# jrnerupudinho/Semi-Blind-Channel-Estimation-for-MIMO-RIS-communication-system-Using-EM-Algo

Hardware: NVIDIA B200
Metric: EM channel-estimation trials/sec (higher is better)
Workload: dtype f64

## Files before the change

### semi-blind-channel-estimation-for-mimo-ris-communication-system-using-em-algo_b200/csrc/abi.cu

```cuda
#include <atomic>
#include <mutex>
#include <vector>
#include <stdio.h>
#include <string.h>

#include "common.cuh"

namespace sbce {

static std::atomic<long long> g_launches{0};
void count_launch(int n) { g_launches.fetch_add(n, std::memory_order_relaxed); }

struct PhaseSpan { int phase; cudaEvent_t a, b; };
static std::atomic<bool> g_prof_on{false};
static std::vector<PhaseSpan> g_spans;
static std::vector<cudaEvent_t> g_event_pool;
static std::mutex g_prof_mu;

static cudaEvent_t prof_event() {
    {
        std::lock_guard<std::mutex> lock(g_prof_mu);
        if (!g_event_pool.empty()) { cudaEvent_t e = g_event_pool.back(); g_event_pool.pop_back(); return e; }
    }
    cudaEvent_t e;
    cudaEventCreate(&e);
    return e;
}

struct PhaseScope {
    bool on; int phase; cudaStream_t s; cudaEvent_t a;
    PhaseScope(int ph, cudaStream_t st) : on(g_prof_on.load(std::memory_order_relaxed)), phase(ph), s(st), a(nullptr) {
        if (on) { a = prof_event(); cudaEventRecord(a, s); }
    }
    ~PhaseScope() {
        if (on) {
            cudaEvent_t b = prof_event();
            cudaEventRecord(b, s);
            std::lock_guard<std::mutex> lock(g_prof_mu);
            g_spans.push_back({phase, a, b});
        }
    }
};

static int make_dims(const sbce_cfg* c, Dims* d, bool with_estep = true) {
    if (!c) return SBCE_E_NULL;
    if (c->N < 1 || c->n_tx < 1 || c->n_rx < 1 || c->T_p < 0 || c->T_d < 1 || c->itera < 0 || c->batch < 0)
        return SBCE_E_SHAPE;
    int sq = 0;
    if (c->M == 4) sq = 2; else if (c->M == 16) sq = 4; else if (c->M == 64) sq = 8; else return SBCE_E_UNSUPPORTED;
    if (c->n_tx > 8 || c->n_rx > 8) return SBCE_E_UNSUPPORTED;
    if (!gram_supports(c->N + 1, c->n_tx, c->n_rx)) return SBCE_E_UNSUPPORTED;
    if (c->n_tx <= 4 && !(c->n_rx <= 4 || c->n_rx == 6 || c->n_rx == 8)) return SBCE_E_UNSUPPORTED;
    if (c->mode < SBCE_MODE_SOFT || c->mode > SBCE_MODE_MMSE) return SBCE_E_UNSUPPORTED;
    if (with_estep) {
        const int log2M = sq == 2 ? 2 : (sq == 4 ? 4 : 6), bits = c->n_tx * log2M;
        const bool tree = c->mode == SBCE_MODE_SOFT || c->mode == SBCE_MODE_HARD;
        if (tree && !enum_instantiated(c->n_tx, log2M)) return SBCE_E_UNSUPPORTED;
        if ((c->mode == SBCE_MODE_ZF || c->mode == SBCE_MODE_MMSE) && bits > 30) return SBCE_E_UNSUPPORTED;
    }
    d->N = c->N; d->N1 = c->N + 1; d->n_tx = c->n_tx; d->n_rx = c->n_rx; d->M = c->M; d->sqM = sq;
    d->bitsM = (sq == 2 ? 2 : (sq == 4 ? 4 : 6));
    d->T_p = c->T_p; d->T_d = c->T_d; d->itera = c->itera;
    d->L = d->N1 * c->n_tx;
    d->Lp = (d->L + 7) & ~7;
    d->RP = (c->n_rx + 3) & ~3;
    d->Ltot = d->Lp + d->RP;
    d->mode = c->mode; d->flags = c->flags; d->p1 = c->partition_p1;
    d->psi_shared = (c->flags & SBCE_FLAG_PSI_SHARED) ? 1 : 0;
    d->psiP_shared = (c->flags & (SBCE_FLAG_PSI_SHARED | SBCE_FLAG_PSIP_SHARED)) ? 1 : 0;
    d->rec = qr_record_doubles(c->n_tx);
    if (c->mode == SBCE_MODE_PM || c->mode == SBCE_MODE_PM_BETA) {
        if (c->partition_p1 < 1 || c->partition_p1 > c->n_tx) return SBCE_E_SHAPE;
        if (with_estep && c->partition_p1 * d->bitsM > 24) return SBCE_E_UNSUPPORTED;
    }
    if (c->mode >= SBCE_MODE_PM && c->n_rx < c->n_tx) return SBCE_E_UNSUPPORTED;
    if (c->flags & SBCE_FLAG_SUPERIMPOSED) {
        if (c->T_p != 0) return SBCE_E_SHAPE;
        if (c->mode != SBCE_MODE_SOFT && c->mode != SBCE_MODE_HARD) return SBCE_E_UNSUPPORTED;
    }
    return 0;
}

static inline size_t al(size_t x) { return (x + 255) & ~(size_t)255; }

size_t carve_workspace(const Dims& d, int nb, void* base, Workspace* ws) {
    size_t off = 0;
    char* p = (char*)base;
    auto take = [&](size_t bytes) { char* r = p ? p + off : nullptr; off += al(bytes); return r; };
    const size_t B = (size_t)nb;
    ws->stat_m = (double*)take(B * d.T_d * d.n_tx * 16);
    ws->stat_R = (double*)take(B * d.T_d * d.n_tx * d.n_tx * 16);
    ws->pil_m = (double*)take(B * d.T_p * d.n_tx * 16 + 16);
    ws->pil_R = (double*)take(B * d.T_p * d.n_tx * d.n_tx * 16 + 16);
    ws->qr = (double*)take(B * d.T_d * d.rec * 8);
    ws->lse_sym = (double*)take(B * d.T_d * 8);
    ws->Gp = (double*)take(B * d.Ltot * d.Lp * 16);
    ws->G = (double*)take(B * d.Ltot * d.Lp * 16);
    ws->active = (int32_t*)take(B * 4);
    ws->stat = (int32_t*)take(B * 4);
    ws->kscratch = (int32_t*)take(B * d.T_d * 4);
    ws->thbuf = (double*)take(B * d.Lp * d.n_rx * 16);
    ws->psiw = (double*)take(B * d.T_p * d.N1 * 16 + 16);
    ws->ls_scale = (double*)take(B * d.N1 * 8);
    ws->ls_rep = (int32_t*)take(B * d.N1 * 4);
    ws->bytes = off;
    return off;
}

#define CK(x)                                  \
    do {                                       \
        cudaError_t _e = (x);                  \
        if (_e != cudaSuccess) return (int)_e; \
    } while (0)

cudaError_t launch_pm_stats(const Dims& d, int nb, const double* Yd, const double* PsiD, const double* theta,
                            const double* varn, const int32_t* active, double* stat_m, double* stat_R,
                            int32_t* kstar, cudaStream_t s);

static int estep_dispatch(const Dims& d, int nb, const double* Yd, const double* PsiD, const double* theta,
                          const double* varn, const int32_t* active, Workspace& ws, double* stat_m, double* stat_R,
                          int32_t* kstar, double* lse_sym, const double* Xoff, cudaStream_t s) {
    if (d.mode == SBCE_MODE_SOFT || d.mode == SBCE_MODE_HARD) {
        {
            PhaseScope ps(SBCE_PHASE_HEFF_QR, s);
            CK(launch_heff_qr(d, nb, Yd, PsiD, theta, active, Xoff, ws.qr, s));
        }
        {
            PhaseScope ps(SBCE_PHASE_ENUM, s);
            CK(launch_enum(d, nb, ws.qr, varn, active, stat_m, stat_R, kstar, lse_sym, s));
            if (Xoff) CK(launch_superimpose_stats(d, nb, Xoff, active, stat_m, stat_R, s));
        }
    } else {
        PhaseScope ps(SBCE_PHASE_ENUM, s);
        CK(launch_pm_stats(d, nb, Yd, PsiD, theta, varn, active, stat_m, stat_R, kstar, s));
    }
    return 0;
}

static inline Dims pilot_dims(const Dims& d) { Dims dp = d; dp.psi_shared = d.psiP_shared; return dp; }

static int em_chunk(const Dims& d, int nb, const sbce_io& io, Workspace& ws, cudaStream_t s) {
    const bool tree = d.mode == SBCE_MODE_SOFT || d.mode == SBCE_MODE_HARD;
    const bool decides = tree || d.mode == SBCE_MODE_ZF || d.mode == SBCE_MODE_MMSE;
    if (io.kstar && !decides) CK(cudaMemsetAsync(io.kstar, 0xFF, (size_t)nb * d.T_d * sizeof(int32_t), s));
    {
        PhaseScope ps(SBCE_PHASE_SETUP, s);
        CK(launch_init_state(d, nb, io.theta0, io.theta, ws.active, ws.stat, io.iters, io.llf, io.lse, s));
        CK(launch_pilot_stats(d, nb, io.Xp, ws.pil_m, ws.pil_R, s));
        CK(launch_normal_equations(pilot_dims(d), nb, io.PsiP, d.T_p, io.Yp, ws.pil_m, ws.pil_R, nullptr, ws.Gp, nullptr, s));
    }
    for (int l = 0; l < d.itera; ++l) {
        int rc = estep_dispatch(d, nb, io.Yd, io.PsiD, io.theta, io.varn, ws.active, ws, ws.stat_m, ws.stat_R,
                                io.kstar, ws.lse_sym, (d.flags & SBCE_FLAG_SUPERIMPOSED) ? io.Xp : nullptr, s);
        if (rc) return rc;
        {
            PhaseScope ps(SBCE_PHASE_GRAM, s);
            CK(launch_normal_equations(d, nb, io.PsiD, d.T_d, io.Yd, ws.stat_m, ws.stat_R, ws.Gp, ws.G, ws.active,
                                       s));
        }
        {
            PhaseScope ps(SBCE_PHASE_CHOL, s);
            CK(launch_chol_solve(d, nb, ws.G, io.theta, ws.active, ws.stat, ws.thbuf, s));
        }
        {
            PhaseScope ps(SBCE_PHASE_METRICS, s);
            CK(launch_after_iteration(d, nb, l, io.theta, io.h_true, io.Yp, io.Yd, io.PsiP, io.PsiD, io.Xp,
                                      io.Xd_true, io.varn, tree ? ws.lse_sym : nullptr, ws.active, io.iters, io.llf,
                                      io.lse, s));
        }
    }
    {
        PhaseScope ps(SBCE_PHASE_METRICS, s);
        CK(launch_final_metrics(d, nb, io.theta, io.h_true, ws.stat, io.nmse, io.status, s));
    }
    return 0;
}

static sbce_io offset_io(const Dims& d, const sbce_io& io, size_t b0) {
    sbce_io o = io;
    const size_t Ln = (size_t)d.L * d.n_rx * 2;
    auto adv = [](const double* p, size_t n) { return p ? p + n : p; };
    auto advw = [](double* p, size_t n) { return p ? p + n : p; };
    o.Yd = adv(io.Yd, b0 * d.T_d * d.n_rx * 2);
    o.Yp = adv(io.Yp, b0 * d.T_p * d.n_rx * 2);
    if (!d.psi_shared) o.PsiD = adv(io.PsiD, b0 * d.T_d * d.N1 * 2);
    if (!d.psiP_shared) o.PsiP = adv(io.PsiP, b0 * d.T_p * d.N1 * 2);
    o.Xp = adv(io.Xp, b0 * ((d.flags & SBCE_FLAG_SUPERIMPOSED) ? d.T_d : d.T_p) * d.n_tx * 2);
    o.theta0 = adv(io.theta0, b0 * Ln);
    o.varn = adv(io.varn, b0);
    o.h_true = adv(io.h_true, b0 * Ln);
    o.Xd_true = adv(io.Xd_true, b0 * d.T_d * d.n_tx * 2);
    o.theta = advw(io.theta, b0 * Ln);
    o.kstar = io.kstar ? io.kstar + b0 * d.T_d : nullptr;
    o.llf = advw(io.llf, b0 * d.itera);
    o.lse = advw(io.lse, b0 * d.itera);
    o.nmse = advw(io.nmse, b0);
    o.iters = io.iters ? io.iters + b0 : nullptr;
    o.status = io.status ? io.status + b0 : nullptr;
    return o;
}

static int check_io(const Dims& d, const sbce_io* io) {
    if (!io) return SBCE_E_NULL;
    if (!io->Yd || !io->PsiD || !io->varn || !io->theta) return SBCE_E_NULL;
    if (d.T_p > 0 && (!io->Yp || !io->PsiP || !io->Xp)) return SBCE_E_NULL;
    if (!(d.flags & SBCE_FLAG_ZERO_START) && !io->theta0) return SBCE_E_NULL;
    if ((d.flags & SBCE_FLAG_GENIE_STOP) && !io->h_true) return SBCE_E_NULL;
    if ((d.flags & SBCE_FLAG_SUPERIMPOSED) && !io->Xp) return SBCE_E_NULL;
    return 0;
}

}

using namespace sbce;

extern "C" {

int sbce_version(void) { return SBCE_VERSION; }

const char* sbce_error_string(int code) {
    switch (code) {
        case 0: return "ok";
        case SBCE_E_NULL: return "required pointer is null";
        case SBCE_E_SHAPE: return "invalid shape parameter";
        case SBCE_E_UNSUPPORTED: return "unsupported configuration (n_tx,n_rx<=8; n_tx<=4: n_rx in {1,2,3,4,6,8}; M in {4,16,64}; N+1+n_tx^2<=908; exhaustive modes with n_tx>4 need n_tx*log2(M)<=24; PM modes need partition_p1*log2(M)<=24)";
        case SBCE_E_WORKSPACE: return "workspace too small for one trial";
        case SBCE_E_NODEVICE: return "no CUDA device";
        default: return code > 0 ? cudaGetErrorString((cudaError_t)code) : "unknown error";
    }
}

int sbce_device_count(void) {
    int n = 0;
    if (cudaGetDeviceCount(&n) != cudaSuccess) { cudaGetLastError(); return 0; }
    return n;
}

int sbce_workspace_bytes(const sbce_cfg* cfg, int32_t trials_in_flight, size_t* bytes) {
    Dims d;
    int rc = make_dims(cfg, &d);
    if (rc) return rc;
    if (!bytes) return SBCE_E_NULL;
    if (trials_in_flight < 1) return SBCE_E_SHAPE;
    Workspace ws;
    *bytes = carve_workspace(d, trials_in_flight, nullptr, &ws);
    return 0;
}

constexpr int SBCE_MAX_CHUNK = 65535;
static int trials_fitting(const Dims& d, size_t bytes, int want) {
    Workspace ws;
    if (want > SBCE_MAX_CHUNK) want = SBCE_MAX_CHUNK;
    if (carve_workspace(d, 1, nullptr, &ws) > bytes) return 0;
    int lo = 1, hi = want;
    while (lo < hi) {
        int mid = (lo + hi + 1) / 2;
        if (carve_workspace(d, mid, nullptr, &ws) <= bytes) lo = mid; else hi = mid - 1;
    }
    return lo;
}

int sbce_em_batch(const sbce_cfg* cfg, const sbce_io* io, void* workspace, size_t workspace_bytes, void* stream) {
    Dims d;
    int rc = make_dims(cfg, &d);
    if (rc) return rc;
    rc = check_io(d, io);
    if (rc) return rc;
    if (cfg->batch == 0) return 0;
    if (!workspace) return SBCE_E_NULL;
    const int chunk = trials_fitting(d, workspace_bytes, cfg->batch);
    if (chunk < 1) return SBCE_E_WORKSPACE;
    cudaStream_t s = (cudaStream_t)stream;
    for (int b0 = 0; b0 < cfg->batch; b0 += chunk) {
        const int nb = (cfg->batch - b0 < chunk) ? cfg->batch - b0 : chunk;
        Workspace ws;
        carve_workspace(d, nb, workspace, &ws);
        sbce_io o = offset_io(d, *io, (size_t)b0);
        rc = em_chunk(d, nb, o, ws, s);
        if (rc) return rc;
    }
    return 0;
}
// ... 392 lines not shown
```

### semi-blind-channel-estimation-for-mimo-ris-communication-system-using-em-algo_b200/csrc/common.cuh

```cuda
#pragma once

#include <cuda_runtime.h>
#include <stdint.h>

#include <atomic>

#include "../../include/sbce.h"

namespace sbce {

typedef double2 cplx;

__host__ __device__ __forceinline__ cplx mk(double re, double im) { return make_double2(re, im); }
__device__ __forceinline__ cplx cadd(cplx a, cplx b) { return mk(a.x + b.x, a.y + b.y); }
__device__ __forceinline__ cplx csub(cplx a, cplx b) { return mk(a.x - b.x, a.y - b.y); }
__device__ __forceinline__ cplx cmul(cplx a, cplx b) {
    return mk(fma(a.x, b.x, -a.y * b.y), fma(a.x, b.y, a.y * b.x));
}
__device__ __forceinline__ cplx cmulc(cplx a, cplx b) {
    return mk(fma(a.x, b.x, a.y * b.y), fma(a.y, b.x, -a.x * b.y));
}
__device__ __forceinline__ cplx cconj(cplx a) { return mk(a.x, -a.y); }
__device__ __forceinline__ cplx cscale(cplx a, double s) { return mk(a.x * s, a.y * s); }
__device__ __forceinline__ double cnorm2(cplx a) { return fma(a.x, a.x, a.y * a.y); }
__device__ __forceinline__ void cfma(cplx& acc, cplx a, cplx b) {
    acc.x = fma(a.x, b.x, acc.x);
    acc.x = fma(-a.y, b.y, acc.x);
    acc.y = fma(a.x, b.y, acc.y);
    acc.y = fma(a.y, b.x, acc.y);
}
__device__ __forceinline__ void cfmac(cplx& acc, cplx a, cplx b) {
    acc.x = fma(a.x, b.x, acc.x);
    acc.x = fma(a.y, b.y, acc.x);
    acc.y = fma(a.y, b.x, acc.y);
    acc.y = fma(-a.x, b.y, acc.y);
}
__device__ __forceinline__ void cfmsc(cplx& acc, cplx a, cplx b) {
    acc.x = fma(-a.x, b.x, acc.x);
    acc.x = fma(-a.y, b.y, acc.x);
    acc.y = fma(-a.y, b.x, acc.y);
    acc.y = fma(a.x, b.y, acc.y);
}

__device__ __forceinline__ double shfl_xor_d(double v, int m) { return __shfl_xor_sync(0xffffffffu, v, m); }
__device__ __forceinline__ double shfl_d(double v, int src) { return __shfl_sync(0xffffffffu, v, src); }
__device__ __forceinline__ double warp_sum(double v) {
#pragma unroll
    for (int o = 16; o > 0; o >>= 1) v += shfl_xor_d(v, o);
    return v;
}

constexpr int RH_MAXR = 8;

struct Dims {
    int N, N1, n_tx, n_rx, M, sqM, bitsM, T_p, T_d, itera;
    int L;
    int Lp;
    int RP;
    int Ltot;
    int mode;
    unsigned flags;
    int p1;
    int psi_shared;
    int psiP_shared;
    int rec;
};

__host__ __device__ __forceinline__ constexpr int qr_rec_R(int n_tx, int i, int j) {
    return 2 * (i * n_tx - i * (i - 1) / 2 + j - i);
}
__host__ __device__ __forceinline__ constexpr int qr_rec_yt(int n_tx, int i) { return n_tx * (n_tx + 1) + 2 * i; }
__host__ __device__ __forceinline__ constexpr int qr_rec_c0(int n_tx) { return qr_rec_yt(n_tx, n_tx); }
__host__ __device__ __forceinline__ constexpr int qr_record_doubles(int n_tx) { return n_tx * (n_tx + 1) + 2 * n_tx + 2; }
static_assert(qr_rec_yt(8, 0) == qr_rec_R(8, 7, 7) + 2 && qr_rec_c0(8) + 2 == qr_record_doubles(8),
              "QR record: R, ytilde and c0 are packed back to back");

constexpr bool enum_instantiated(int n_tx, int log2M) { return n_tx <= 4 || n_tx * log2M <= 24; }

struct Workspace {
    double* stat_m;
    double* stat_R;
    double* pil_m;
    double* pil_R;
    double* qr;
    double* lse_sym;
    double* Gp;
    double* G;
    int32_t* active;
    int32_t* stat;
    int32_t* kscratch;
    double* psiw;
    double* ls_scale;
    int32_t* ls_rep;
    double* thbuf;
    size_t bytes;
};

size_t carve_workspace(const Dims& d, int nb, void* base, Workspace* ws);

cudaError_t launch_pilot_stats(const Dims& d, int nb, const double* Xp, double* pil_m, double* pil_R, cudaStream_t s);
cudaError_t launch_heff_qr(const Dims& d, int nb, const double* Yd, const double* PsiD, const double* theta,
                           const int32_t* active, const double* Xoff, double* qr, cudaStream_t s);
cudaError_t launch_superimpose_stats(const Dims& d, int nb, const double* Xoff, const int32_t* active, double* stat_m,
                                     double* stat_R, cudaStream_t s);
cudaError_t launch_enum(const Dims& d, int nb, const double* qr, const double* varn, const int32_t* active,
                        double* stat_m, double* stat_R, int32_t* kstar, double* lse_sym, cudaStream_t s);
cudaError_t launch_normal_equations(const Dims& d, int nb, const double* Psi, int T, const double* Y,
                                    const double* sm, const double* sR, const double* Ginit, double* Gout,
                                    const int32_t* active, cudaStream_t s);
bool gram_supports(int N1, int n_tx, int n_rx);
cudaError_t launch_chol_solve(const Dims& d, int nb, double* G, double* theta, const int32_t* active, int32_t* stat,
                              double* th_scratch, cudaStream_t s);
cudaError_t launch_init_state(const Dims& d, int nb, const double* theta0, double* theta, int32_t* active,
                              int32_t* stat, int32_t* iters, double* llf, double* lse, cudaStream_t s);
cudaError_t launch_after_iteration(const Dims& d, int nb, int l, const double* theta, const double* h_true,
                                   const double* Yp, const double* Yd, const double* PsiP, const double* PsiD,
                                   const double* Xp, const double* Xd_true, const double* varn, const double* lse_sym,
                                   int32_t* active, int32_t* iters, double* llf, double* lse, cudaStream_t s);
cudaError_t launch_final_metrics(const Dims& d, int nb, const double* theta, const double* h_true, const int32_t* stat,
                                 double* nmse, int32_t* status, cudaStream_t s);
cudaError_t launch_accumulate_nmse(const double* nmse, const int32_t* status, int batch, double* acc, cudaStream_t s);
cudaError_t run_fp64_peak(double* tflops, double* seconds);
cudaError_t launch_generate(const Dims& d, int nb, const sbce_gen* g, const sbce_io& io, double* h_out, double* Xp_out,
                            double* Xd_out, double* PsiP_out, double* PsiD_out, double* Yp_out, double* Yd_out,
                            cudaStream_t s);
cudaError_t launch_ls_start(const Dims& d, int nb, const sbce_io& io, double* theta0, int32_t* status, Workspace& ws,
                            cudaStream_t s);
cudaError_t launch_accumulate_ser(const Dims& d, int nb, const int32_t* kstar, const double* Xd, double* acc,
                                  cudaStream_t s);

void count_launch(int n = 1);


struct SmemOptIn {
    std::atomic<size_t> have[64];
};
inline cudaError_t opt_in_smem(SmemOptIn& st, const void* kernel, size_t smem) {
    if (smem <= 48 * 1024) return cudaSuccess;
    int dev = 0;
    cudaError_t e = cudaGetDevice(&dev);
    if (e != cudaSuccess) return e;
    if (dev >= 0 && dev < 64 && st.have[dev].load(std::memory_order_relaxed) >= smem) return cudaSuccess;
    e = cudaFuncSetAttribute(kernel, cudaFuncAttributeMaxDynamicSharedMemorySize, (int)smem);
    if (e == cudaSuccess && dev >= 0 && dev < 64) st.have[dev].store(smem, std::memory_order_relaxed);
    return e;
}

}
```

### semi-blind-channel-estimation-for-mimo-ris-communication-system-using-em-algo_b200/csrc/estep.cu

```cuda
#include <math.h>

#include "common.cuh"
#include "tensor.cuh"

namespace sbce {

static __device__ __forceinline__ constexpr int cmax(int a, int b) { return a > b ? a : b; }

__global__ void k_pilot_stats(int n_tx, int total, const cplx* __restrict__ Xp, cplx* __restrict__ pm,
                              cplx* __restrict__ pR) {
    int s = blockIdx.x * blockDim.x + threadIdx.x;
    if (s >= total) return;
    const cplx* x = Xp + (size_t)s * n_tx;
    for (int i = 0; i < n_tx; ++i) {
        cplx xi = x[i];
        pm[(size_t)s * n_tx + i] = cconj(xi);
        for (int j = 0; j < n_tx; ++j) pR[((size_t)s * n_tx + i) * n_tx + j] = cmulc(x[j], xi);
    }
}

cudaError_t launch_pilot_stats(const Dims& d, int nb, const double* Xp, double* pil_m, double* pil_R, cudaStream_t s) {
    int total = nb * d.T_p;
    if (total == 0) return cudaSuccess;
    k_pilot_stats<<<(total + 127) / 128, 128, 0, s>>>(d.n_tx, total, (const cplx*)Xp, (cplx*)pil_m, (cplx*)pil_R);
// ... 526 lines not shown
        }
        __syncwarp(hm);
    }
    __syncwarp(hm);
    if (lane == 0) ws[E::O_AREF] = aref;
    __syncwarp(hm);
}

template <int NTX, int SQM, bool HARD>
struct Scan {
    typedef EnumT<NTX, SQM> E;
    static constexpr int M = E::M;
    double* ws;
    const cplx* tab;
    const double* g;
    double r0;
    double thr;
    double best, lim;
    int bestk;
    int cnt;
    bool prune;

    __device__ __forceinline__ void leaf(cplx t0, double nb, int code, bool live) {
        const double fI = E::fold(t0.x, r0), fQ = E::fold(t0.y, r0);
        const double nodemin = fma(fI, fI, fma(fQ, fQ, nb));
        const bool hit = live && nodemin <= lim;
        if (hit && nodemin <= best) {
            double dI, dQ;
            const int iI = E::slice(t0.x, g, dI), iQ = E::slice(t0.y, g, dQ);
            const double val = nb + dI + dQ;
            const int k = code + ((iQ * SQM + iI) << (E::BITS * (NTX - 1)));
            if (val < best || (val == best && k < bestk)) {
                best = val;
                bestk = k;
                lim = HARD ? val : val + thr;
            }
        }
        if (!HARD) {
            const unsigned q = __ballot_sync(E::gmask(), hit) >> E::gshift();
            if (q != 0u) {
                if (hit) {
                    const int slot = cnt + __popc(q & ((1u << E::glane()) - 1u));
                    if (slot < E::QCAP) ((int*)(ws + E::O_Q))[slot] = code;
                }
                cnt += __popc(q);
            }
        }
    }

    __device__ __forceinline__ void merge_best() {
        const unsigned hm = E::gmask();
#pragma unroll
        for (int o = E::G / 2; o > 0; o >>= 1) {
            const double ob = shfl_xor_h(hm, best, o);
            const int ok = __shfl_xor_sync(hm, bestk, o);
            if (ob < best || (ob == best && ok < bestk)) { best = ob; bestk = ok; }
        }
        lim = HARD ? best : best + thr;
    }

    template <int PER_LANE>
    __device__ __forceinline__ void maybe_flush() {
        if (!HARD && cnt > E::QCAP - E::G * PER_LANE) {
            const unsigned hm = E::gmask();
            double wb = best;
#pragma unroll
            for (int o = E::G / 2; o > 0; o >>= 1) wb = fmin(wb, shfl_xor_h(hm, wb, o));
            enum_flush<NTX, SQM>(ws, wb, cnt);
            cnt = 0;
        }
    }


    template <int S_>
    __device__ __forceinline__ void inner(const cplx (&acc)[NTX], double base, int code, cplx r01, bool dead) {
        dead = dead || (prune && base > lim);
        if constexpr (S_ == 0) {
            leaf(acc[0], base, code, !dead);
        } else if constexpr (S_ == 1 && M % E::G == 0) {
            const unsigned hm = E::gmask();
            unsigned todo = __ballot_sync(hm, !dead) >> E::gshift();
            while (todo != 0u) {
                const int src = __ffs(todo) - 1;
                todo &= todo - 1u;
                cplx pacc[NTX];
#pragma unroll
                for (int i = 0; i < NTX; ++i)
                    pacc[i] = i <= 1 ? mk(__shfl_sync(hm, acc[i].x, src, E::G), __shfl_sync(hm, acc[i].y, src, E::G))
                                     : acc[i];
                const double pbase = __shfl_sync(hm, base, src, E::G);
                const int pcode = __shfl_sync(hm, code, src, E::G);
#pragma unroll 1
                for (int m = E::glane(); m < M; m += E::G) {
                    cplx nacc[NTX];
                    const double nb = E::step(pacc, nacc, 1, m, pbase, g, tab);
                    const double b0 = best;
                    inner<0>(nacc, nb, pcode + (m << (E::BITS * (NTX - 2))), r01, false);
                    if (__any_sync(hm, best != b0)) merge_best();
                    maybe_flush<1>();
                }
            }
        } else if constexpr (S_ == 1) {
            if (__all_sync(E::gmask(), dead)) return;
            constexpr bool NODE_FLUSH = E::G * M < E::QCAP;
            const double* g1 = g + SQM;
            double dI1[SQM];
#pragma unroll
            for (int a = 0; a < SQM; ++a) {
                const double eI = acc[1].x - g1[a];
                dI1[a] = eI * eI;
            }
#pragma unroll 1
            for (int iQ = 0; iQ < SQM; ++iQ) {
                const double eQ = acc[1].y - g1[iQ];
                const double bq = base + __dmul_rn(eQ, eQ);
                const bool deadq = dead || (prune && bq > lim);
                if (__all_sync(E::gmask(), deadq)) continue;
                const double pQ = E::pam(iQ);
                const cplx tq = mk(fma(pQ, r01.y, acc[0].x), fma(-pQ, r01.x, acc[0].y));
                const int cq = code + ((iQ * SQM) << (E::BITS * (NTX - 2)));
#pragma unroll
                for (int iI = 0; iI < SQM; ++iI) {
                    const double pI = E::pam(iI);
                    const cplx t0 = mk(fma(-pI, r01.x, tq.x), fma(-pI, r01.y, tq.y));
                    leaf(t0, bq + dI1[iI], cq + (iI << (E::BITS * (NTX - 2))), !deadq);
                }
                if (!NODE_FLUSH) maybe_flush<SQM>();
            }
            if (NODE_FLUSH) maybe_flush<M>();
        } else {
            if (__all_sync(E::gmask(), dead)) return;
#pragma unroll 1
            for (int m = 0; m < M; ++m) {
                cplx nacc[NTX];
                const double nb = E::step(acc, nacc, S_, m, base, g, tab);
                inner<S_ - 1>(nacc, nb, code + (m << (E::BITS * (NTX - 1 - S_))), r01, dead);
            }
        }
    }

    template <int S_, int LEFT>
    __device__ __forceinline__ void prefix(const cplx (&acc)[NTX], double base, int code, int p, cplx r01, bool dead) {
        if constexpr (LEFT == 0) {
            inner<S_>(acc, base, code, r01, dead);
        } else {
            const int m = (p >> (E::BITS * (LEFT - 1))) & (M - 1);
            cplx nacc[NTX];
            const double nb = E::step(acc, nacc, S_, m, base, g, tab);
            prefix<S_ - 1, LEFT - 1>(nacc, nb, code + (m << (E::BITS * (NTX - 1 - S_))), p, r01, dead);
        }
    }
};

template <int NTX, int SQM, bool HARD, int WARPS>
__global__ void __launch_bounds__(WARPS * 32, (NTX > 4 ? 2 : 4)) k_enum(Dims d, const double* __restrict__ qr,
                                                     const double* __restrict__ varn,
                                                     const int32_t* __restrict__ active, cplx* __restrict__ stat_m,
                                                     cplx* __restrict__ stat_R, int32_t* __restrict__ kstar,
                                                     double* __restrict__ lse_sym) {
    typedef EnumT<NTX, SQM> E;
    constexpr int M = E::M;
    extern __shared__ __align__(16) double enum_smem[];
    const int b = blockIdx.y;
    constexpr int SPW = 32 / E::G;
    const int warp = threadIdx.x >> 5, sub = (threadIdx.x & 31) / E::G, gl = E::glane();
    const int t = (blockIdx.x * WARPS + warp) * SPW + sub;
    if (t >= d.T_d) return;
    const double* grec = qr + ((size_t)b * d.T_d + t) * d.rec;
    const int32_t act = (active != nullptr) ? active[b] : 1;
    const double vn = varn[b];
    const double rec0 = (gl < E::REC) ? grec[gl] : 0.0;
    if (act == 0) return;

    double* ws = enum_smem + (size_t)(SPW * warp + sub) * E::WS_DOUBLES;
    cplx* tab = (cplx*)(ws + E::O_TAB);
    double* g = ws + E::O_G;
    const double* rec = ws + E::O_SCR;
    {
        if (gl < E::REC) ws[E::O_SCR + gl] = rec0;
        for (int i = gl + E::G; i < E::REC; i += E::G) ws[E::O_SCR + i] = grec[i];
        __syncwarp(E::gmask());
    }
    cplx yt[NTX];
    cplx r01 = mk(0.0, 0.0);
    double r00;
    {
        cplx Rm[NTX][NTX];
#pragma unroll
        for (int i = 0; i < NTX; ++i)
#pragma unroll
            for (int j = i; j < NTX; ++j) Rm[i][j] = mk(rec[qr_rec_R(NTX, i, j)], rec[qr_rec_R(NTX, i, j) + 1]);
#pragma unroll
        for (int i = 0; i < NTX; ++i) yt[i] = mk(rec[qr_rec_yt(NTX, i)], rec[qr_rec_yt(NTX, i) + 1]);
        r00 = Rm[0][0].x;
        if (NTX > 1) r01 = Rm[0][NTX > 1 ? 1 : 0];
#pragma unroll
        for (int s = 1; s < NTX; ++s)
#pragma unroll
            for (int i = 0; i < s; ++i)
                for (int m = gl; m < M; m += E::G) tab[E::pair(i, s) * M + m] = cmul(Rm[i][s], E::cval(m));
        if (gl < SQM) {
#pragma unroll
            for (int s = 0; s < NTX; ++s) g[s * SQM + gl] = Rm[s][s].x * E::pam(gl);
        }
    }
    const double c0 = rec[qr_rec_c0(NTX)];
    const double s2 = vn * vn, inv_s2 = 1.0 / s2;
    if (gl == 0) {
#pragma unroll
        for (int i = 0; i < NTX; ++i) {
            ws[E::O_YT + 2 * i] = yt[i].x;
            ws[E::O_YT + 2 * i + 1] = yt[i].y;
        }
        ws[E::O_C0] = c0;
        ws[E::O_AREF] = 1e300;
        ws[E::O_S2] = inv_s2;
    }
    for (int i = gl; i < E::NACC; i += E::G) ws[E::O_ACC + i] = 0.0;
    __syncwarp(E::gmask());

    Scan<NTX, SQM, HARD> sc;
    sc.ws = ws;
    sc.tab = tab;
    sc.g = g;
    sc.r0 = r00;
    sc.thr = SBCE_THR * s2;
    sc.cnt = 0;
    sc.prune = (d.flags & SBCE_FLAG_FULL_SCAN) == 0;
    {
        cplx acc[NTX];
#pragma unroll
        for (int i = 0; i < NTX; ++i) acc[i] = yt[i];
        double base = c0;
        int k = 0;
#pragma unroll
        for (int s = NTX - 1; s >= 0; --s) {
            double dI, dQ;
            const int iI = E::slice(acc[s].x, g + s * SQM, dI), iQ = E::slice(acc[s].y, g + s * SQM, dQ);
            const int m = iQ * SQM + iI;
            base += dI + dQ;
            k += m << (E::BITS * (NTX - 1 - s));
            E::descend(acc, acc, s, m, tab);
        }
        sc.best = base;
        sc.bestk = k;
        sc.lim = HARD ? base : base + sc.thr;
    }

    constexpr int NROUND = (E::NPREF + E::G - 1) / E::G;
    static_assert(NROUND <= 32, "one bit per round");
    unsigned live = NROUND == 32 ? 0xffffffffu : (1u << NROUND) - 1u;
    if (E::PL >= 2 && sc.prune) {
        constexpr int TOP_SHIFT = E::BITS * (E::PL - 1);
        const bool a = gl < M && !(c0 + E::dist(yt, NTX - 1, gl, g) > sc.lim);
        const unsigned top_alive = __ballot_sync(E::gmask(), a) >> E::gshift();
        live = 0u;
#pragma unroll
        for (int r = 0; r < NROUND; ++r) {
            const int lo = (E::G * r) >> TOP_SHIFT, hi = min(E::G * r + E::G - 1, E::NPREF - 1) >> TOP_SHIFT;
            const unsigned bits = ((2u << hi) - 1u) & ~((1u << lo) - 1u);
            if (top_alive & bits) live |= 1u << r;
        }
    }
    while (live != 0u) {
        const int pb = E::G * (__ffs(live) - 1);
        live &= live - 1u;
        const int p = pb + gl;
        const bool valid = p < E::NPREF;
        cplx acc[NTX];
#pragma unroll
        for (int i = 0; i < NTX; ++i) acc[i] = mk(ws[E::O_YT + 2 * i], ws[E::O_YT + 2 * i + 1]);
        sc.template prefix<NTX - 1, E::PL>(acc, ws[E::O_C0], 0, valid ? p : 0, r01, !valid);
    }

    sc.merge_best();
    const double best = sc.best;
    const int bestk = sc.bestk;
    const size_t sidx = (size_t)b * d.T_d + t;
    if (kstar != nullptr && gl == 0) kstar[sidx] = bestk;

    bool collapsed = HARD;
    double S = 0.0;
    if (!HARD) {
        enum_flush<NTX, SQM>(ws, best, sc.cnt);
        S = ws[E::O_ACC];
        if (!(S > 0.0) || !isfinite(S)) collapsed = true;
    }
    if (collapsed) {
        if (gl == 0) {
            cplx xs[NTX];
#pragma unroll
            for (int s = 0; s < NTX; ++s) xs[s] = E::cval(E::digit(bestk, s));
#pragma unroll
            for (int i = 0; i < NTX; ++i) {
                stat_m[sidx * NTX + i] = cconj(xs[i]);
#pragma unroll
                for (int j = 0; j < NTX; ++j) stat_R[(sidx * NTX + i) * NTX + j] = cmulc(xs[j], xs[i]);
            }
            if (lse_sym != nullptr) lse_sym[sidx] = -best * inv_s2;
        }
        return;
    }
    {
        const double invS = 1.0 / S;
        const double* A = ws + E::O_ACC;
        for (int l = gl; l < NTX * NTX; l += E::G) {
            const int i = l / NTX, j = l % NTX;
            cplx v;
            if (i == j) {
                v = mk(A[E::A_RD + j] * invS, 0.0);
            } else {
                const int pr = E::acc_R(min(i, j), max(i, j));
                const double a = A[pr] * invS, c = A[pr + 1] * invS;
                v = mk(a, i < j ? c : -c);
            }
            stat_R[sidx * NTX * NTX + l] = v;
        }
        if (gl < NTX) stat_m[sidx * NTX + gl] = mk(A[E::A_MRE + gl] * invS, A[E::A_MIM + gl] * invS);
        if (lse_sym != nullptr && gl == 0) lse_sym[sidx] = -ws[E::O_AREF] * inv_s2 + log(S);
    }
}

__global__ void k_superimpose_stats(Dims d, int nb, const cplx* __restrict__ Xoff, const int32_t* __restrict__ active,
                                    cplx* __restrict__ stat_m, cplx* __restrict__ stat_R) {
    const int s = blockIdx.x * blockDim.x + threadIdx.x;
    if (s >= nb * d.T_d) return;
    if (active != nullptr && active[s / d.T_d] == 0) return;
    const int n = d.n_tx;
    const cplx* o = Xoff + (size_t)s * n;
    cplx* m = stat_m + (size_t)s * n;
    cplx* R = stat_R + (size_t)s * n * n;
    for (int i = 0; i < n; ++i)
        for (int j = 0; j < n; ++j) {
            cplx v = R[i * n + j];
            cfma(v, m[i], o[j]);
            v = cadd(v, cconj(cmul(o[i], m[j])));
            v = cadd(v, cmulc(o[j], o[i]));
            R[i * n + j] = v;
        }
    for (int i = 0; i < n; ++i) m[i] = cadd(m[i], cconj(o[i]));
}

cudaError_t launch_superimpose_stats(const Dims& d, int nb, const double* Xoff, const int32_t* active, double* stat_m,
                                     double* stat_R, cudaStream_t s) {
    const int total = nb * d.T_d;
    k_superimpose_stats<<<(total + 127) / 128, 128, 0, s>>>(d, nb, (const cplx*)Xoff, active, (cplx*)stat_m, (cplx*)stat_R);
    count_launch();
    return cudaGetLastError();
}

template <int NTX, int NRX>
static cudaError_t run_heff(const Dims& d, int nb, const double* Yd, const double* PsiD, const double* theta,
                            const int32_t* active, const double* Xoff, double* qr, cudaStream_t s) {
    static SmemOptIn optin_mma, optin;
    dim3 grid((d.T_d + 127) / 128, nb);
    constexpr int NC = NTX * NRX, NT = (NC + 7) / 8;
    const int KP = (d.N1 + 7) & ~7;
    const size_t smem_mma = sizeof(cplx) * ((size_t)KP * (NT * 8 + 2) + 4 * 32 * (NC + 1));
    if (NC >= 8 && d.N1 >= 16 && smem_mma <= 100 * 1024) {
        cudaError_t e = opt_in_smem(optin_mma, (const void*)k_heff_qr_mma<NTX, NRX>, smem_mma);
        if (e != cudaSuccess) return e;
        k_heff_qr_mma<NTX, NRX><<<grid, 128, smem_mma, s>>>(d, (const cplx*)Yd, (const cplx*)PsiD, (const cplx*)theta,
                                                            active, (const cplx*)Xoff, qr);
        count_launch();
        return cudaGetLastError();
    }
    size_t smem = sizeof(cplx) * (size_t)d.L * NRX;
    const int use_smem = smem <= 64 * 1024;
    if (!use_smem) smem = 0;
    cudaError_t e = opt_in_smem(optin, (const void*)k_heff_qr<NTX, NRX>, smem);
    if (e != cudaSuccess) return e;
    k_heff_qr<NTX, NRX><<<grid, 128, smem, s>>>(d, (const cplx*)Yd, (const cplx*)PsiD, (const cplx*)theta, active,
                                                (const cplx*)Xoff, qr, use_smem);
    count_launch();
    return cudaGetLastError();
}

template <int NTX>
static cudaError_t run_heff_ntx(const Dims& d, int nb, const double* Yd, const double* PsiD, const double* theta,
                                const int32_t* active, const double* Xoff, double* qr, cudaStream_t s) {
    switch (d.n_rx) {
        case 1: return run_heff<NTX, 1>(d, nb, Yd, PsiD, theta, active, Xoff, qr, s);
        case 2: return run_heff<NTX, 2>(d, nb, Yd, PsiD, theta, active, Xoff, qr, s);
        case 3: return run_heff<NTX, 3>(d, nb, Yd, PsiD, theta, active, Xoff, qr, s);
        case 4: return run_heff<NTX, 4>(d, nb, Yd, PsiD, theta, active, Xoff, qr, s);
        case 6: return run_heff<NTX, 6>(d, nb, Yd, PsiD, theta, active, Xoff, qr, s);
        case 8: return run_heff<NTX, 8>(d, nb, Yd, PsiD, theta, active, Xoff, qr, s);
        default: return cudaErrorInvalidValue;
    }
}

template <int NTX, int SQM>
static cudaError_t run_enum_sqm(const Dims& d, int nb, const double* qr, const double* varn, const int32_t* active,
                                double* stat_m, double* stat_R, int32_t* kstar, double* lse_sym, cudaStream_t s) {
    typedef EnumT<NTX, SQM> E;
    constexpr int WARPS = 4, SYMS = WARPS * 32 / E::G;
    dim3 grid((d.T_d + SYMS - 1) / SYMS, nb);
    constexpr size_t smem = sizeof(double) * SYMS * E::WS_DOUBLES;
    static SmemOptIn optin[2];
    const bool hard = d.mode == SBCE_MODE_HARD;
    const auto kernel = hard ? k_enum<NTX, SQM, true, WARPS> : k_enum<NTX, SQM, false, WARPS>;
    cudaError_t e = opt_in_smem(optin[hard], (const void*)kernel, smem);
    if (e != cudaSuccess) return e;
    kernel<<<grid, WARPS * 32, smem, s>>>(d, qr, varn, active, (cplx*)stat_m, (cplx*)stat_R, kstar, lse_sym);
    count_launch();
    return cudaGetLastError();
}

template <int NTX>
static cudaError_t run_enum(const Dims& d, int nb, const double* qr, const double* varn, const int32_t* active,
                            double* stat_m, double* stat_R, int32_t* kstar, double* lse_sym, cudaStream_t s) {
    switch (d.sqM) {
        case 2:
            if constexpr (enum_instantiated(NTX, 2))
                return run_enum_sqm<NTX, 2>(d, nb, qr, varn, active, stat_m, stat_R, kstar, lse_sym, s);
            break;
        case 4:
            if constexpr (enum_instantiated(NTX, 4))
                return run_enum_sqm<NTX, 4>(d, nb, qr, varn, active, stat_m, stat_R, kstar, lse_sym, s);
            break;
        case 8:
            if constexpr (enum_instantiated(NTX, 6))
                return run_enum_sqm<NTX, 8>(d, nb, qr, varn, active, stat_m, stat_R, kstar, lse_sym, s);
            break;
    }
    return cudaErrorInvalidValue;
}

template <int NTX>
static cudaError_t run_heff_rows(const Dims& d, int nb, const double* Yd, const double* PsiD, const double* theta,
                                 const int32_t* active, const double* Xoff, double* qr, cudaStream_t s) {
    dim3 grid((d.T_d + 15) / 16, nb);
    k_heff_qr_rows<NTX><<<grid, 128, 0, s>>>(d, (const cplx*)Yd, (const cplx*)PsiD, (const cplx*)theta, active,
                                             (const cplx*)Xoff, qr);
    count_launch();
    return cudaGetLastError();
}

cudaError_t launch_heff_qr(const Dims& d, int nb, const double* Yd, const double* PsiD, const double* theta,
                           const int32_t* active, const double* Xoff, double* qr, cudaStream_t s) {
    switch (d.n_tx) {
        case 1: return run_heff_ntx<1>(d, nb, Yd, PsiD, theta, active, Xoff, qr, s);
        case 2: return run_heff_ntx<2>(d, nb, Yd, PsiD, theta, active, Xoff, qr, s);
        case 3: return run_heff_ntx<3>(d, nb, Yd, PsiD, theta, active, Xoff, qr, s);
        case 4: return run_heff_ntx<4>(d, nb, Yd, PsiD, theta, active, Xoff, qr, s);
        case 5: return run_heff_rows<5>(d, nb, Yd, PsiD, theta, active, Xoff, qr, s);
        case 6: return run_heff_rows<6>(d, nb, Yd, PsiD, theta, active, Xoff, qr, s);
        case 7: return run_heff_rows<7>(d, nb, Yd, PsiD, theta, active, Xoff, qr, s);
        case 8: return run_heff_rows<8>(d, nb, Yd, PsiD, theta, active, Xoff, qr, s);
        default: return cudaErrorInvalidValue;
    }
}

cudaError_t launch_enum(const Dims& d, int nb, const double* qr, const double* varn, const int32_t* active,
                        double* stat_m, double* stat_R, int32_t* kstar, double* lse_sym, cudaStream_t s) {
    switch (d.n_tx) {
        case 1: return run_enum<1>(d, nb, qr, varn, active, stat_m, stat_R, kstar, lse_sym, s);
        case 2: return run_enum<2>(d, nb, qr, varn, active, stat_m, stat_R, kstar, lse_sym, s);
        case 3: return run_enum<3>(d, nb, qr, varn, active, stat_m, stat_R, kstar, lse_sym, s);
        case 4: return run_enum<4>(d, nb, qr, varn, active, stat_m, stat_R, kstar, lse_sym, s);
        case 5: return run_enum<5>(d, nb, qr, varn, active, stat_m, stat_R, kstar, lse_sym, s);
        case 6: return run_enum<6>(d, nb, qr, varn, active, stat_m, stat_R, kstar, lse_sym, s);
        case 7: return run_enum<7>(d, nb, qr, varn, active, stat_m, stat_R, kstar, lse_sym, s);
        case 8: return run_enum<8>(d, nb, qr, varn, active, stat_m, stat_R, kstar, lse_sym, s);
        default: return cudaErrorInvalidValue;
    }
}

}
```

Before: 25280.

## Make enumeration kernel persistent with atomic work-claiming across warps

Replaces the per-symbol grid launch of the sphere/enumeration E-step kernel with a persistent grid sized to resident CTAs, where each warp claims work units (a trial and a group of symbols) through a global atomic counter. The goal is to balance the highly variable per-symbol enumeration cost (from pruning) across SMs and cut tail imbalance. The per-symbol body moves into a noinline device function that prefetches the next claim early. In exchange it adds a memset plus atomic contention per launch and a function-call boundary that may cost registers.

```diff
diff --git a/semi-blind-channel-estimation-for-mimo-ris-communication-system-using-em-algo_b200/csrc/abi.cu b/semi-blind-channel-estimation-for-mimo-ris-communication-system-using-em-algo_b200/csrc/abi.cu
--- a/semi-blind-channel-estimation-for-mimo-ris-communication-system-using-em-algo_b200/csrc/abi.cu
+++ b/semi-blind-channel-estimation-for-mimo-ris-communication-system-using-em-algo_b200/csrc/abi.cu
@@ -103,6 +103,7 @@
     ws->psiw = (double*)take(B * d.T_p * d.N1 * 16 + 16);
     ws->ls_scale = (double*)take(B * d.N1 * 8);
     ws->ls_rep = (int32_t*)take(B * d.N1 * 4);
+    ws->enum_claims = (int32_t*)take(4);
     ws->bytes = off;
     return off;
 }
@@ -127,7 +128,7 @@
         }
         {
             PhaseScope ps(SBCE_PHASE_ENUM, s);
-            CK(launch_enum(d, nb, ws.qr, varn, active, stat_m, stat_R, kstar, lse_sym, s));
+            CK(launch_enum(d, nb, ws.qr, varn, active, stat_m, stat_R, kstar, lse_sym, ws.enum_claims, s));
             if (Xoff) CK(launch_superimpose_stats(d, nb, Xoff, active, stat_m, stat_R, s));
         }
     } else {
diff --git a/semi-blind-channel-estimation-for-mimo-ris-communication-system-using-em-algo_b200/csrc/common.cuh b/semi-blind-channel-estimation-for-mimo-ris-communication-system-using-em-algo_b200/csrc/common.cuh
--- a/semi-blind-channel-estimation-for-mimo-ris-communication-system-using-em-algo_b200/csrc/common.cuh
+++ b/semi-blind-channel-estimation-for-mimo-ris-communication-system-using-em-algo_b200/csrc/common.cuh
@@ -93,6 +93,7 @@
     double* ls_scale;
     int32_t* ls_rep;
     double* thbuf;
+    int32_t* enum_claims;
     size_t bytes;
 };
 
@@ -104,7 +105,8 @@
 cudaError_t launch_superimpose_stats(const Dims& d, int nb, const double* Xoff, const int32_t* active, double* stat_m,
                                      double* stat_R, cudaStream_t s);
 cudaError_t launch_enum(const Dims& d, int nb, const double* qr, const double* varn, const int32_t* active,
-                        double* stat_m, double* stat_R, int32_t* kstar, double* lse_sym, cudaStream_t s);
+                        double* stat_m, double* stat_R, int32_t* kstar, double* lse_sym, int32_t* claims,
+                        cudaStream_t s);
 cudaError_t launch_normal_equations(const Dims& d, int nb, const double* Psi, int T, const double* Y,
                                     const double* sm, const double* sR, const double* Ginit, double* Gout,
                                     const int32_t* active, cudaStream_t s);
diff --git a/semi-blind-channel-estimation-for-mimo-ris-communication-system-using-em-algo_b200/csrc/estep.cu b/semi-blind-channel-estimation-for-mimo-ris-communication-system-using-em-algo_b200/csrc/estep.cu
--- a/semi-blind-channel-estimation-for-mimo-ris-communication-system-using-em-algo_b200/csrc/estep.cu
+++ b/semi-blind-channel-estimation-for-mimo-ris-communication-system-using-em-algo_b200/csrc/estep.cu
@@ -702,33 +702,32 @@
     }
 };
 
-template <int NTX, int SQM, bool HARD, int WARPS>
-__global__ void __launch_bounds__(WARPS * 32, (NTX > 4 ? 2 : 4)) k_enum(Dims d, const double* __restrict__ qr,
-                                                     const double* __restrict__ varn,
-                                                     const int32_t* __restrict__ active, cplx* __restrict__ stat_m,
-                                                     cplx* __restrict__ stat_R, int32_t* __restrict__ kstar,
-                                                     double* __restrict__ lse_sym) {
+template <int NTX, int SQM, bool HARD>
+__device__ __noinline__ int enum_symbol(int b, size_t sidx, int rec_len, bool prune, double* ws, const double* __restrict__ qr,
+                                        const double* __restrict__ varn, const int32_t* __restrict__ active,
+                                        cplx* __restrict__ stat_m, cplx* __restrict__ stat_R,
+                                        int32_t* __restrict__ kstar, double* __restrict__ lse_sym,
+                                        int32_t* __restrict__ claims) {
     typedef EnumT<NTX, SQM> E;
     constexpr int M = E::M;
-    extern __shared__ __align__(16) double enum_smem[];
-    const int b = blockIdx.y;
-    constexpr int SPW = 32 / E::G;
-    const int warp = threadIdx.x >> 5, sub = (threadIdx.x & 31) / E::G, gl = E::glane();
-    const int t = (blockIdx.x * WARPS + warp) * SPW + sub;
-    if (t >= d.T_d) return;
-    const double* grec = qr + ((size_t)b * d.T_d + t) * d.rec;
+    const int gl = E::glane();
+    const int next = (threadIdx.x & 31) == 0 ? atomicAdd(claims, 1) : 0;
+    constexpr int NR = (E::REC + E::G - 1) / E::G;
+    const double* grec = qr + sidx * rec_len;
     const int32_t act = (active != nullptr) ? active[b] : 1;
     const double vn = varn[b];
-    const double rec0 = (gl < E::REC) ? grec[gl] : 0.0;
-    if (act == 0) return;
-
-    double* ws = enum_smem + (size_t)(SPW * warp + sub) * E::WS_DOUBLES;
+    double r[NR];
+#pragma unroll
+    for (int i = 0; i < NR; ++i) r[i] = (gl + E::G * i < E::REC) ? grec[gl + E::G * i] : 0.0;
+    if (act == 0) return next;
+
     cplx* tab = (cplx*)(ws + E::O_TAB);
     double* g = ws + E::O_G;
     const double* rec = ws + E::O_SCR;
     {
-        if (gl < E::REC) ws[E::O_SCR + gl] = rec0;
-        for (int i = gl + E::G; i < E::REC; i += E::G) ws[E::O_SCR + i] = grec[i];
+#pragma unroll
+        for (int i = 0; i < NR; ++i)
+            if (gl + E::G * i < E::REC) ws[E::O_SCR + gl + E::G * i] = r[i];
         __syncwarp(E::gmask());
     }
     cplx yt[NTX];
@@ -776,7 +775,7 @@
     sc.r0 = r00;
     sc.thr = SBCE_THR * s2;
     sc.cnt = 0;
-    sc.prune = (d.flags & SBCE_FLAG_FULL_SCAN) == 0;
+    sc.prune = prune;
     {
         cplx acc[NTX];
 #pragma unroll
@@ -826,7 +825,6 @@
     sc.merge_best();
     const double best = sc.best;
     const int bestk = sc.bestk;
-    const size_t sidx = (size_t)b * d.T_d + t;
     if (kstar != nullptr && gl == 0) kstar[sidx] = bestk;
 
     bool collapsed = HARD;
@@ -849,7 +847,7 @@
             }
             if (lse_sym != nullptr) lse_sym[sidx] = -best * inv_s2;
         }
-        return;
+        return next;
     }
     {
         const double invS = 1.0 / S;
@@ -868,6 +866,32 @@
         }
         if (gl < NTX) stat_m[sidx * NTX + gl] = mk(A[E::A_MRE + gl] * invS, A[E::A_MIM + gl] * invS);
         if (lse_sym != nullptr && gl == 0) lse_sym[sidx] = -ws[E::O_AREF] * inv_s2 + log(S);
+    }
+    return next;
+}
+
+template <int NTX, int SQM, bool HARD, int WARPS>
+__global__ void __launch_bounds__(WARPS * 32, (NTX > 4 ? 2 : 4)) k_enum(Dims d, int nb, const double* __restrict__ qr,
+                                                     const double* __restrict__ varn,
+                                                     const int32_t* __restrict__ active, cplx* __restrict__ stat_m,
+                                                     cplx* __restrict__ stat_R, int32_t* __restrict__ kstar,
+                                                     double* __restrict__ lse_sym, int32_t* __restrict__ claims) {
+    typedef EnumT<NTX, SQM> E;
+    extern __shared__ __align__(16) double enum_smem[];
+    constexpr int SPW = 32 / E::G;
+    const int warp = threadIdx.x >> 5, lane = threadIdx.x & 31, sub = lane / E::G;
+    double* ws = enum_smem + (size_t)(SPW * warp + sub) * E::WS_DOUBLES;
+    const int per_trial = (d.T_d + SPW - 1) / SPW, nclaim = nb * per_trial;
+    const bool prune = (d.flags & SBCE_FLAG_FULL_SCAN) == 0;
+    int j = __shfl_sync(0xffffffffu, lane == 0 ? atomicAdd(claims, 1) : 0, 0);
+    while (j < nclaim) {
+        const int b = j / per_trial, t = (j - b * per_trial) * SPW + sub;
+        int next = 0;
+        if (t < d.T_d)
+            next = enum_symbol<NTX, SQM, HARD>(b, (size_t)b * d.T_d + t, d.rec, prune, ws, qr, varn, active, stat_m,
+                                               stat_R, kstar, lse_sym, claims);
+        __syncwarp();
+        j = __shfl_sync(0xffffffffu, next, 0);
     }
 }
 
@@ -940,38 +964,66 @@
     }
 }
 
+struct ResidentCtas {
+    std::atomic<int> n[64];
+};
+static cudaError_t resident_ctas(ResidentCtas& st, const void* kernel, int threads, size_t smem, int* ctas) {
+    int dev = 0;
+    cudaError_t e = cudaGetDevice(&dev);
+    if (e != cudaSuccess) return e;
+    if (dev >= 0 && dev < 64 && (*ctas = st.n[dev].load(std::memory_order_relaxed)) > 0) return cudaSuccess;
+    int per_sm = 0, sms = 0;
+    e = cudaOccupancyMaxActiveBlocksPerMultiprocessor(&per_sm, kernel, threads, smem);
+    if (e == cudaSuccess) e = cudaDeviceGetAttribute(&sms, cudaDevAttrMultiProcessorCount, dev);
+    if (e != cudaSuccess) return e;
+    if (per_sm < 1) return cudaErrorInvalidConfiguration;
+    *ctas = per_sm * sms;
+    if (dev >= 0 && dev < 64) st.n[dev].store(*ctas, std::memory_order_relaxed);
+    return cudaSuccess;
+}
+
 template <int NTX, int SQM>
 static cudaError_t run_enum_sqm(const Dims& d, int nb, const double* qr, const double* varn, const int32_t* active,
-                                double* stat_m, double* stat_R, int32_t* kstar, double* lse_sym, cudaStream_t s) {
+                                double* stat_m, double* stat_R, int32_t* kstar, double* lse_sym, int32_t* claims,
+                                cudaStream_t s) {
     typedef EnumT<NTX, SQM> E;
-    constexpr int WARPS = 4, SYMS = WARPS * 32 / E::G;
-    dim3 grid((d.T_d + SYMS - 1) / SYMS, nb);
-    constexpr size_t smem = sizeof(double) * SYMS * E::WS_DOUBLES;
+    constexpr int WARPS = 4, SPW = 32 / E::G;
+    constexpr size_t smem = sizeof(double) * WARPS * SPW * E::WS_DOUBLES;
     static SmemOptIn optin[2];
+    static ResidentCtas resident[2];
     const bool hard = d.mode == SBCE_MODE_HARD;
     const auto kernel = hard ? k_enum<NTX, SQM, true, WARPS> : k_enum<NTX, SQM, false, WARPS>;
     cudaError_t e = opt_in_smem(optin[hard], (const void*)kernel, smem);
     if (e != cudaSuccess) return e;
-    kernel<<<grid, WARPS * 32, smem, s>>>(d, qr, varn, active, (cplx*)stat_m, (cplx*)stat_R, kstar, lse_sym);
+    int ctas = 0;
+    e = resident_ctas(resident[hard], (const void*)kernel, WARPS * 32, smem, &ctas);
+    if (e != cudaSuccess) return e;
+    const long long warps_needed = (long long)nb * ((d.T_d + SPW - 1) / SPW);
+    if (warps_needed < (long long)ctas * WARPS) ctas = (int)((warps_needed + WARPS - 1) / WARPS);
+    e = cudaMemsetAsync(claims, 0, sizeof(int32_t), s);
+    if (e != cudaSuccess) return e;
+    kernel<<<ctas, WARPS * 32, smem, s>>>(d, nb, qr, varn, active, (cplx*)stat_m, (cplx*)stat_R, kstar, lse_sym,
+                                          claims);
     count_launch();
     return cudaGetLastError();
 }
 
 template <int NTX>
 static cudaError_t run_enum(const Dims& d, int nb, const double* qr, const double* varn, const int32_t* active,
-                            double* stat_m, double* stat_R, int32_t* kstar, double* lse_sym, cudaStream_t s) {
+                            double* stat_m, double* stat_R, int32_t* kstar, double* lse_sym, int32_t* claims,
+                            cudaStream_t s) {
     switch (d.sqM) {
         case 2:
             if constexpr (enum_instantiated(NTX, 2))
-                return run_enum_sqm<NTX, 2>(d, nb, qr, varn, active, stat_m, stat_R, kstar, lse_sym, s);
+                return run_enum_sqm<NTX, 2>(d, nb, qr, varn, active, stat_m, stat_R, kstar, lse_sym, claims, s);
             break;
         case 4:
             if constexpr (enum_instantiated(NTX, 4))
-                return run_enum_sqm<NTX, 4>(d, nb, qr, varn, active, stat_m, stat_R, kstar, lse_sym, s);
+                return run_enum_sqm<NTX, 4>(d, nb, qr, varn, active, stat_m, stat_R, kstar, lse_sym, claims, s);
             break;
         case 8:
             if constexpr (enum_instantiated(NTX, 6))
-                return run_enum_sqm<NTX, 8>(d, nb, qr, varn, active, stat_m, stat_R, kstar, lse_sym, s);
+                return run_enum_sqm<NTX, 8>(d, nb, qr, varn, active, stat_m, stat_R, kstar, lse_sym, claims, s);
             break;
     }
     return cudaErrorInvalidValue;
@@ -1003,16 +1055,17 @@
 }
 
 cudaError_t launch_enum(const Dims& d, int nb, const double* qr, const double* varn, const int32_t* active,
-                        double* stat_m, double* stat_R, int32_t* kstar, double* lse_sym, cudaStream_t s) {
+                        double* stat_m, double* stat_R, int32_t* kstar, double* lse_sym, int32_t* claims,
+                        cudaStream_t s) {
     switch (d.n_tx) {
-        case 1: return run_enum<1>(d, nb, qr, varn, active, stat_m, stat_R, kstar, lse_sym, s);
-        case 2: return run_enum<2>(d, nb, qr, varn, active, stat_m, stat_R, kstar, lse_sym, s);
-        case 3: return run_enum<3>(d, nb, qr, varn, active, stat_m, stat_R, kstar, lse_sym, s);
-        case 4: return run_enum<4>(d, nb, qr, varn, active, stat_m, stat_R, kstar, lse_sym, s);
-        case 5: return run_enum<5>(d, nb, qr, varn, active, stat_m, stat_R, kstar, lse_sym, s);
-        case 6: return run_enum<6>(d, nb, qr, varn, active, stat_m, stat_R, kstar, lse_sym, s);
-        case 7: return run_enum<7>(d, nb, qr, varn, active, stat_m, stat_R, kstar, lse_sym, s);
-        case 8: return run_enum<8>(d, nb, qr, varn, active, stat_m, stat_R, kstar, lse_sym, s);
+        case 1: return run_enum<1>(d, nb, qr, varn, active, stat_m, stat_R, kstar, lse_sym, claims, s);
+        case 2: return run_enum<2>(d, nb, qr, varn, active, stat_m, stat_R, kstar, lse_sym, claims, s);
+        case 3: return run_enum<3>(d, nb, qr, varn, active, stat_m, stat_R, kstar, lse_sym, claims, s);
+        case 4: return run_enum<4>(d, nb, qr, varn, active, stat_m, stat_R, kstar, lse_sym, claims, s);
+        case 5: return run_enum<5>(d, nb, qr, varn, active, stat_m, stat_R, kstar, lse_sym, claims, s);
+        case 6: return run_enum<6>(d, nb, qr, varn, active, stat_m, stat_R, kstar, lse_sym, claims, s);
+        case 7: return run_enum<7>(d, nb, qr, varn, active, stat_m, stat_R, kstar, lse_sym, claims, s);
+        case 8: return run_enum<8>(d, nb, qr, varn, active, stat_m, stat_R, kstar, lse_sym, claims, s);
         default: return cudaErrorInvalidValue;
     }
 }
```

Result: faster. 25680, median of 6 (+1.6%).
